# caki35/UNet-Torch

Measured on AMD Instinct MI355X. Metric: images/sec training step, 4-level U-Net 1ch→2cls 512×512, at 1/2/4/8 MI355X, higher is better.
Workload: dtype f16

## Files before the change

unet-torch_amd/csrc/kernels.h:

```cpp
#pragma once
#include "common.h"

struct ConvFwdProblem {
    int N, H, W, Ci, Co, R, S, stride, pad, Ho, Wo, ldx, ldy, in_dtype, out_dtype, flags;
    bool has_tx, has_bias, has_stats;
};
enum ConvFwdPath { FWD_MFMA3X3_F32, FWD_GEMM_F32, FWD_CONVT_F32, FWD_MFMA3X3, FWD_MFMA1X1, FWD_STEM, FWD_HEAD, FWD_SMALLK, FWD_ROOT, FWD_HEAD3, FWD_GENERIC };

bool umi_conv3x3_f32_mfma_ok(const ConvFwdProblem& p);
bool umi_gemm_f32_mfma_ok(const ConvFwdProblem& p);
bool umi_convt_f32_mfma_ok(const ConvFwdProblem& p);
bool umi_conv3x3_mfma_ok(const ConvFwdProblem& p);
bool umi_conv1x1_mfma_ok(const ConvFwdProblem& p);
bool umi_stem_fwd_ok(const ConvFwdProblem& p);
bool umi_head_fwd_ok(const ConvFwdProblem& p);
bool umi_smallk_fwd_ok(const ConvFwdProblem& p);
bool umi_root_fwd_ok(const ConvFwdProblem& p);
bool umi_head3_fwd_ok(const ConvFwdProblem& p);

constexpr int UMI_CONV_F32_OPT_IN = UMI_CONV_F32_MFMA | UMI_CONV_F32_MFMA_1X1 | UMI_CONV_F32_MFMA_2X2;
inline ConvFwdPath umi_conv_fwd_path(const ConvFwdProblem& p) {
    if (p.flags & UMI_CONV_F32_OPT_IN) {
        if (umi_conv3x3_f32_mfma_ok(p)) return FWD_MFMA3X3_F32;
        if (umi_gemm_f32_mfma_ok(p)) return FWD_GEMM_F32;
// ... 50 lines not shown
int umi_smallk_fwd_bnred(const void* x, int ldx, const void* wp, void* y, int ldy, const void* ybn, int ldybn, const void* txbn,
                         const float* rstd, float* part, long P, int Ci, int Co, hipStream_t s, float* dW = nullptr, long s_co = 0,
                         long s_ci = 0, float out_scale = 1.f, void* ws = nullptr, size_t ws_bytes = 0);
int umi_root_fwd(const ConvFwdProblem& p, const void* x, const void* wp, void* y, hipStream_t s);
int umi_head3_fwd(const ConvFwdProblem& p, const void* x, const void* tx, const void* wp, const float* bias, void* y,
                  hipStream_t s);

struct WgradProblem {
    int N, H, W, Ci, Co, R, S, stride, pad, Ho, Wo, ldx, lddy, dtype, flags;
    bool has_txa, has_txb;
};
struct WgradOut {
    float* dW; long s_co, s_ci, s_t; float out_scale;
    void* ws; size_t ws_bytes;
    umi_wgrad_pending* defer;
    float* convT_bias;
};
struct WgradBnApply { const void* y; int ldy; const void* tx_bn; const float *rstd, *sum_dz, *sum_dzx; void* dz; int lddz;
                      long count; };
enum WgradPath { WGRAD_MFMA3X3_F32, WGRAD_GEMM_F32, WGRAD_CONVT_F32, WGRAD_MFMA3X3, WGRAD_MFMA1X1, WGRAD_T, WGRAD_GATHER, WGRAD_STEM, WGRAD_HEAD, WGRAD_ROOT, WGRAD_HEAD3, WGRAD_GENERIC };

bool umi_wgrad3x3_f32_mfma_ok(const WgradProblem& p);
bool umi_wgrad_gemm_f32_mfma_ok(const WgradProblem& p);
bool umi_wgrad_convt_f32_mfma_ok(const WgradProblem& p);
bool umi_wgrad3x3_mfma_ok(const WgradProblem& p);
bool umi_wgrad1x1_mfma_ok(const WgradProblem& p);
bool umi_wgradT_mfma_ok(const WgradProblem& p);
bool umi_wgrad_gather_mfma_ok(const WgradProblem& p);
bool umi_stem_wgrad_ok(const WgradProblem& p);
bool umi_head_wgrad_ok(const WgradProblem& p);
bool umi_root_wgrad_ok(const WgradProblem& p);
bool umi_head3_wgrad_ok(const WgradProblem& p);

inline WgradPath umi_conv_wgrad_path(const WgradProblem& p) {
    if (p.flags & UMI_CONV_F32_OPT_IN) {
        if (umi_wgrad3x3_f32_mfma_ok(p)) return WGRAD_MFMA3X3_F32;
        if (umi_wgrad_gemm_f32_mfma_ok(p)) return WGRAD_GEMM_F32;
        if (umi_wgrad_convt_f32_mfma_ok(p)) return WGRAD_CONVT_F32;
        WgradProblem q = p;
        q.flags &= ~UMI_CONV_F32_OPT_IN;
        return umi_conv_wgrad_path(q);
    }
    if (umi_wgrad3x3_mfma_ok(p)) return WGRAD_MFMA3X3;
    if (umi_wgrad1x1_mfma_ok(p)) return WGRAD_MFMA1X1;
    if (umi_wgradT_mfma_ok(p)) return WGRAD_T;
    if (umi_wgrad_gather_mfma_ok(p)) return WGRAD_GATHER;
    if (umi_stem_wgrad_ok(p)) return WGRAD_STEM;
    if (umi_head_wgrad_ok(p)) return WGRAD_HEAD;
    if (umi_root_wgrad_ok(p)) return WGRAD_ROOT;
    if (umi_head3_wgrad_ok(p)) return WGRAD_HEAD3;
    return WGRAD_GENERIC;
}

size_t umi_wgrad3x3_f32_mfma_ws_bound(const WgradProblem& p);
size_t umi_wgrad_gemm_f32_mfma_ws_bound(const WgradProblem& p);
size_t umi_wgrad_convt_f32_mfma_ws_bound(const WgradProblem& p);
size_t umi_wgrad3x3_mfma_ws_bound(const WgradProblem& p);
size_t umi_wgrad1x1_mfma_ws_bound(const WgradProblem& p);
size_t umi_wgradT_mfma_ws_bound(const WgradProblem& p);
size_t umi_wgrad_gather_mfma_ws_bound(const WgradProblem& p);
size_t umi_stem_wgrad_ws_bound(const WgradProblem& p);
size_t umi_head_wgrad_ws_bound(const WgradProblem& p);
size_t umi_root_wgrad_ws_bound(const WgradProblem& p);
size_t umi_head3_wgrad_ws_bound(const WgradProblem& p);
size_t umi_conv_wgrad_generic_ws_bound(const WgradProblem& p);

// ... 77 lines not shown
```

unet-torch_amd/csrc/wgrad_mfma.hip:

```cpp
#include "kernels.h"
#include <type_traits>
#include <stdlib.h>

typedef _Float16 half8 __attribute__((ext_vector_type(8)));
typedef _Float16 half4 __attribute__((ext_vector_type(4)));
typedef short short4v __attribute__((ext_vector_type(4)));
typedef float floatx16 __attribute__((ext_vector_type(16)));

#ifdef UMI_STAMP
__device__ unsigned long long umi_stamp_buf_w[2048 * 8];
#define UMI_TW(var)                                                                       \
    unsigned long long var;                                                               \
    __builtin_amdgcn_sched_barrier(0);                                                    \
    asm volatile("s_memtime %0\n\ts_waitcnt lgkmcnt(0)" : "=s"(var)::"memory");           \
    __builtin_amdgcn_sched_barrier(0)
extern "C" int umi_debug_read_stamps_w(void* dst) {
    return (int)hipMemcpyFromSymbol(dst, HIP_SYMBOL(umi_stamp_buf_w), sizeof(umi_stamp_buf_w));
}
#endif

namespace {

constexpr int TR = 4;
constexpr int HPIX = (TR + 2) * 34;
// ... 177 lines not shown
#endif
        __syncthreads();
#ifdef UMI_STAMP
        UMI_TW(t4);
        seg[0] += t0b - t0; seg[1] += t1 - t0b; seg[2] += t2 - t1; seg[3] += t3 - t2; seg[4] += t4 - t3;
#endif
    }
#undef UMI_ISSUE
#ifdef UMI_STAMP
    UMI_TW(t_ep0);
#endif

    const int co = co0 + wco * 32 + (lane & 31);
#pragma unroll
    for (int tap = 0; tap < 9; ++tap)
#pragma unroll
        for (int r = 0; r < 16; ++r) {
            int ci = ci0 + wci * 32 + (r & 3) + 8 * (r >> 2) + 4 * (lane >> 5);
            if (ci < Ci && co < Co) part[(((long)blockIdx.y * 9 + tap) * Ci + ci) * Co + co] = acc[tap][r];
        }
#ifdef UMI_STAMP
    UMI_TW(t_end_);
    const int bid = blockIdx.y * gridDim.x + blockIdx.x;
    if (lane == 0 && bid < 512) {
#pragma unroll
        for (int i = 0; i < 5; ++i) umi_stamp_buf_w[(bid * 4 + wave) * 8 + i] = seg[i];
        umi_stamp_buf_w[(bid * 4 + wave) * 8 + 5] = t_end - t_begin;
        umi_stamp_buf_w[(bid * 4 + wave) * 8 + 6] = t_loop - t_start;
        umi_stamp_buf_w[(bid * 4 + wave) * 8 + 7] = t_end_ - t_ep0;
    }
#endif
}

constexpr int WS_SMEM = 2 * SMEM;

struct BnApply {
    const half_t* y; int ldy; const float4* tx; const float* rstd; const float* sum_dz; const float* sum_dzx; long count;
    half_t* dz; int lddz;
};

template <bool HAS_TX, bool BNA>
__global__ __launch_bounds__(512, 1) void wgrad3x3_ws_kernel(
    const half_t* __restrict__ x, int ldx, const float4* __restrict__ tx, const half_t* __restrict__ dy, int lddy,
    float* __restrict__ part, int N, int H, int W, int Ci, int Co, int tiles_x, int tiles_y, int tiles_total,
    int tiles_per_split, int n_co_t, int fast_ci, BnApply ba) {
    extern __shared__ __attribute__((aligned(16))) unsigned char smem_ws[];
    float4* txs = reinterpret_cast<float4*>(smem_ws + WS_SMEM);
    const int tid = threadIdx.x;
    const int lane = tid & 63, wave = tid >> 6;
    const bool producer = wave >= 4;
    const int n_ci_t = (int)gridDim.x / n_co_t;
    const int ci0 = (fast_ci ? (int)blockIdx.x % n_ci_t : (int)blockIdx.x / n_co_t) * 64;
    const int co0 = (fast_ci ? (int)blockIdx.x / n_ci_t : (int)blockIdx.x % n_co_t) * 64;
    const int t_begin = blockIdx.y * tiles_per_split;
    int t_end = t_begin + tiles_per_split;
    if (t_end > tiles_total) t_end = tiles_total;
    const int ntile = t_end - t_begin;
    if (HAS_TX) {
        if (tid < 64) txs[(tid & 7) * 8 + (tid >> 3)] = ci0 + tid < Ci ? tx[ci0 + tid] : make_float4(0.f, 1.f, 0.f, 0.f);
        __syncthreads();
    }

    if (producer) {
        const int ptid = tid - 256;
        const int sub = ptid & 7;
        const bool a_on = ci0 + sub * 8 < Ci, b_on = co0 + sub * 8 < Co;
        constexpr unsigned OOB = 0x7FFFFFFFu;
        int hyx[KPA], aoff[KPA];
#pragma unroll
        for (int k = 0; k < KPA; ++k) {
            int hp = (ptid >> 3) + 32 * k;
            int hy = hp / 34, hx = hp - hy * 34;
            hyx[k] = (hp < HPIX && a_on) ? (int)(((unsigned)(hy - 1) << 16) | ((unsigned)(hx - 1) & 0xffffu)) : (int)0x80000000;
            aoff[k] = (((hy - 1) * W + (hx - 1)) * ldx + ci0 + sub * 8) * 2;
        }
        const bool whole_tiles = (W & 31) == 0 && H % TR == 0;
        const int aback = (W + 1) * ldx * 2;
        int ering[KPA];
        unsigned aoffb[KPA];
#pragma unroll
        for (int k = 0; k < KPA; ++k) {
            int hp = (ptid >> 3) + 32 * k;
            int hy = hp / 34, hx = hp - hy * 34;
            ering[k] = (hp < HPIX && a_on) ? ((hx == 0 ? 1 : 0) | (hx == 33 ? 2 : 0) | (hy == 0 ? 4 : 0) | (hy == TR + 1 ? 8 : 0)) : 16;
            aoffb[k] = (unsigned)(aoff[k] + aback);
        }
        const int bcol = ptid >> 3;
        const int boff0 = (bcol * lddy + co0 + sub * 8) * 2;
        const int a_lds = (sub >> 2) * A_CHUNK + (ptid >> 3) * PROW + (sub & 3) * 16;
        const int b_lds = A_BYTES + (sub >> 2) * B_CHUNK + (ptid >> 3) * PROW + (sub & 3) * 16;
        const long ximg = (long)H * W * ldx, yimg = (long)H * W * lddy;
        float4 t[8];
#pragma unroll
        for (int j = 0; j < 8; ++j) t[j] = HAS_TX ? txs[j * 8 + sub] : make_float4(0.f, 1.f, 0.f, 0.f);
        float4 tb[8];
        float rsb[8], c1[8], c2[8];
        const long ybimg = BNA ? (long)H * W * ba.ldy : 0;
        const int ybo0 = BNA ? (bcol * ba.ldy + co0 + sub * 8) * 2 : 0;
        const bool dz_writer = BNA && ci0 == 0;
        if (BNA) {
            const float invM = 1.f / (float)ba.count;
#pragma unroll
            for (int j = 0; j < 8; ++j) {
                const int c = co0 + sub * 8 + j;
                const bool in = c < Co;
                tb[j] = in ? ba.tx[c] : make_float4(0.f, 1.f, 0.f, 0.f);
                rsb[j] = in ? ba.rstd[c] : 0.f;
                c1[j] = in ? ba.sum_dz[c] * invM : 0.f;
                c2[j] = in ? ba.sum_dzx[c] * invM : 0.f;
            }
        }
        half8 yraw0[KPB], yraw1[KPB];
        bool bvalid0[KPB], bvalid1[KPB];
        int st_n0 = 0, st_y0 = 0, st_x0 = 0, st_n1 = 0, st_y1 = 0, st_x1 = 0;
        half8 araw0[KPA], braw0[KPB], araw1[KPA], braw1[KPB];
        bool avalid0[KPA], avalid1[KPA];
        int nx_n, nx_y, nx_x;
        {
            const int tpi = tiles_x * tiles_y;
            nx_n = t_begin / tpi;
            const int rm = t_begin - nx_n * tpi;
            nx_y = (rm / tiles_x) * TR;
            nx_x = (rm % tiles_x) * 32;
        }
#ifdef UMI_EXP_WS_NO_LOAD
#define UMI_EXP_LOAD_OK(c_) ((c_) && H < 0)
#else
#define UMI_EXP_LOAD_OK(c_) (c_)
#endif
#define UMI_ISSUE_WS(S)                                                                                          \
    do {                                                                                                        \
        const __amdgpu_buffer_rsrc_t xrs = __builtin_amdgcn_make_buffer_rsrc((void*)(x + nx_n * ximg), 0, (int)(ximg * 2), 0x00020000); \
        const __amdgpu_buffer_rsrc_t yrs = __builtin_amdgcn_make_buffer_rsrc((void*)(dy + nx_n * yimg), 0, (int)(yimg * 2), 0x00020000); \
        const int org = nx_y * W + nx_x;                                                                        \
        const unsigned abase = (unsigned)org * (unsigned)(ldx * 2), bbase = (unsigned)org * (unsigned)(lddy * 2);  \
        if (whole_tiles) {                                                                                      \
            const __amdgpu_buffer_rsrc_t xrsb = __builtin_amdgcn_make_buffer_rsrc((void*)((const char*)(x + nx_n * ximg) - aback), 0, (int)(ximg * 2) + aback, 0x00020000); \
            const int edge = (nx_x == 0 ? 1 : 0) | (nx_x + 32 >= W ? 2 : 0) | (nx_y == 0 ? 4 : 0) | (nx_y + TR >= H ? 8 : 0) | 16; \
            _Pragma("unroll") for (int k = 0; k < KPA; ++k) {                                                   \
                avalid##S[k] = (ering[k] & edge) == 0;                                                          \
                araw##S[k] = __builtin_bit_cast(half8, __builtin_amdgcn_raw_buffer_load_b128(                   \
                    xrsb, UMI_EXP_LOAD_OK(avalid##S[k]) ? aoffb[k] : OOB, abase, 0));                           \
            }                                                                                                   \
        } else {                                                                                                \
            _Pragma("unroll") for (int k = 0; k < KPA; ++k) {                                                   \
                const int gy = nx_y + (hyx[k] >> 16), gx = nx_x + (int)(short)(hyx[k] & 0xffff);                \
                avalid##S[k] = hyx[k] != (int)0x80000000 && (unsigned)gy < (unsigned)H && (unsigned)gx < (unsigned)W; \
                araw##S[k] = __builtin_bit_cast(half8, __builtin_amdgcn_raw_buffer_load_b128(                   \
                    xrs, UMI_EXP_LOAD_OK(avalid##S[k]) ? abase + (unsigned)aoff[k] : OOB, 0, 0));               \
            }                                                                                                   \
        }                                                                                                       \
        _Pragma("unroll") for (int k = 0; k < KPB; ++k) {                                                       \
            const bool ok = b_on && (whole_tiles || (nx_y + k < H && nx_x + bcol < W));                         \
            braw##S[k] = __builtin_bit_cast(half8, __builtin_amdgcn_raw_buffer_load_b128(                       \
                yrs, UMI_EXP_LOAD_OK(ok) ? (unsigned)boff0 : OOB, bbase + k * W * lddy * 2, 0));                \
            if (BNA) {                                                                                          \
                const __amdgpu_buffer_rsrc_t ybrs = __builtin_amdgcn_make_buffer_rsrc((void*)(ba.y + nx_n * ybimg), 0, (int)(ybimg * 2), 0x00020000); \
                bvalid##S[k] = ok;                                                                              \
                yraw##S[k] = __builtin_bit_cast(half8, __builtin_amdgcn_raw_buffer_load_b128(                   \
                    ybrs, ok ? (unsigned)org * (unsigned)(ba.ldy * 2) + (unsigned)(ybo0 + k * W * ba.ldy * 2) : OOB, 0, 0)); \
            }                                                                                                   \
        }                                                                                                       \
        if (BNA) { st_n##S = nx_n; st_y##S = nx_y; st_x##S = nx_x; }                                            \
        nx_x += 32;                                                                                             \
        if (nx_x >= W) { nx_x = 0; nx_y += TR; if (nx_y >= H) { nx_y = 0; ++nx_n; } }                           \
    } while (0)
#ifdef UMI_EXP_WS_NO_STORE
#define UMI_STORE_WS(S, buf_)                                                                                    \
    do {                                                                                                        \
        _Pragma("unroll") for (int k = 0; k < KPA; ++k) asm volatile("" ::"v"(araw##S[k]));                     \
        _Pragma("unroll") for (int k = 0; k < KPB; ++k) asm volatile("" ::"v"(braw##S[k]));                     \
    } while (0)
#else
#define UMI_STORE_WS(S, buf_)                                                                                    \
    do {                                                                                                        \
        unsigned char* sb = smem_ws + (buf_) * SMEM;                                                            \
        if (HAS_TX) {                                                                                           \
            _Pragma("unroll") for (int k = 0; k < KPA; ++k) {                                                   \
                const half8 t8 = umi_tx8(araw##S[k], t);                                                        \
                araw##S[k] = avalid##S[k] ? t8 : araw##S[k];       \
            }                                                                                                   \
        }                                                                                                       \
        _Pragma("unroll") for (int k = 0; k < KPA; ++k)                                                         \
            if ((ptid >> 3) + 32 * k < HPIX) *reinterpret_cast<half8*>(sb + a_lds + k * 32 * PROW) = araw##S[k]; \
        if (BNA) {                                                                                              \
            _Pragma("unroll") for (int k = 0; k < KPB; ++k) {                                                   \
                const half8 o = umi_bn_dz8(yraw##S[k], braw##S[k], tb, rsb, c1, c2);    \
                braw##S[k] = bvalid##S[k] ? o : braw##S[k];              \
                if (dz_writer && bvalid##S[k])                                                                  \
                    *reinterpret_cast<half8*>(ba.dz + ((long)((long)st_n##S * H + st_y##S + k) * W + st_x##S + bcol) * ba.lddz + \
                                              co0 + sub * 8) = braw##S[k];                                      \
            }                                                                                                   \
        }                                                                                                       \
        _Pragma("unroll") for (int k = 0; k < KPB; ++k) *reinterpret_cast<half8*>(sb + b_lds + k * 32 * PROW) = braw##S[k]; \
    } while (0)
#endif

        if (ntile > 0) UMI_ISSUE_WS(0);
        if (ntile > 1) UMI_ISSUE_WS(1);
        if (ntile > 0) UMI_STORE_WS(0, 0);
        if (ntile > 2) UMI_ISSUE_WS(0);
        __syncthreads();
#ifdef UMI_STAMP
        unsigned long long pw = 0, pb = 0;
#define UMI_PS(a_) UMI_TW(a_)
#else
#define UMI_PS(a_)
#endif
        for (int i = 0; i < ntile; i += 2) {
            UMI_PS(q0);
#ifndef UMI_EXP_WS_NO_PROD
            if (i + 1 < ntile) {
                UMI_STORE_WS(1, 1);
                if (i + 3 < ntile) UMI_ISSUE_WS(1);
            }
#endif
            UMI_PS(q1);
            __syncthreads();
            UMI_PS(q2);
            if (i + 1 < ntile) {
#ifndef UMI_EXP_WS_NO_PROD
                if (i + 2 < ntile) {
                    UMI_STORE_WS(0, 0);
                    if (i + 4 < ntile) UMI_ISSUE_WS(0);
                }
#endif
                UMI_PS(q3);
                __syncthreads();
                UMI_PS(q4);
#ifdef UMI_STAMP
                pw += q3 - q2; pb += q4 - q3;
#endif
            }
#ifdef UMI_STAMP
            pw += q1 - q0; pb += q2 - q1;
#endif
        }
#ifdef UMI_STAMP
        {
            const int bid = blockIdx.y * gridDim.x + blockIdx.x;
            if (lane == 0 && bid < 256) {
                umi_stamp_buf_w[(bid * 8 + wave) * 8 + 0] = pw;
                umi_stamp_buf_w[(bid * 8 + wave) * 8 + 1] = pb;
                umi_stamp_buf_w[(bid * 8 + wave) * 8 + 5] = ntile;
            }
        }
#endif
#undef UMI_PS
#undef UMI_ISSUE_WS
#undef UMI_STORE_WS
        return;
    }

    __builtin_amdgcn_s_setprio(3);
    const int wci = wave >> 1, wco = wave & 1;
    typedef float floatx4 __attribute__((ext_vector_type(4)));
    floatx4 acc[9][2][2];
#pragma unroll
    for (int t = 0; t < 9; ++t)
#pragma unroll
        for (int ca = 0; ca < 2; ++ca)
#pragma unroll
            for (int cb = 0; cb < 2; ++cb)
#pragma unroll
                for (int r = 0; r < 4; ++r) acc[t][ca][cb][r] = 0.f;
    const int g = lane >> 4, li = lane & 15, lq = li >> 2, lp = li & 3;
    const int frag_lane = (8 * g + lq) * PROW + (4 * lp) * 2;
    __syncthreads();
#define UMI_LD_A16(dst, ca_, dx_)                                                                                \
    _Pragma("unroll") for (int rr = 0; rr < TR + 2; ++rr) dst[rr] = tr_frag(a_frag + (rr * 34 + (dx_)) * PROW + (ca_) * 32)
#define UMI_MMA16(af_, ca_, dx_)                                                                                 \
    _Pragma("unroll") for (int r = 0; r < TR; ++r)                                                              \
        _Pragma("unroll") for (int dyi = 0; dyi < 3; ++dyi)                                                     \
            _Pragma("unroll") for (int cb = 0; cb < 2; ++cb)                                                    \
                acc[dyi * 3 + (dx_)][ca_][cb] = __builtin_amdgcn_mfma_f32_16x16x32_f16(af_[r + dyi], bfr[r][cb], acc[dyi * 3 + (dx_)][ca_][cb], 0, 0, 0)
#define UMI_PIN() __builtin_amdgcn_sched_barrier(0)
#ifdef UMI_STAMP
    unsigned long long cw = 0, cb_ = 0, cstart = 0;
#endif
    for (int i = 0; i < ntile; ++i) {
#ifdef UMI_STAMP
        UMI_TW(c0);
#endif
        const unsigned char* a_frag = smem_ws + (i & 1) * SMEM + wci * A_CHUNK + frag_lane;
        const unsigned char* b_frag = smem_ws + (i & 1) * SMEM + A_BYTES + wco * B_CHUNK + frag_lane;
        half8 a0[TR + 2], a1[TR + 2], bfr[TR][2];
#pragma unroll
        for (int r = 0; r < TR; ++r)
#pragma unroll
            for (int cb = 0; cb < 2; ++cb) bfr[r][cb] = tr_frag(b_frag + (r * 32) * PROW + cb * 32);
#ifndef UMI_WS_COARSE
#define UMI_STEP(ld_, mma_) do { ld_; mma_;                                                              \
            _Pragma("unroll") for (int i_ = 0; i_ < 12; ++i_) {                                                     \
                __builtin_amdgcn_sched_group_barrier(0x008, 2, 0); __builtin_amdgcn_sched_group_barrier(0x100, 1, 0); }  \
            UMI_PIN(); } while (0)
        UMI_LD_A16(a0, 0, 0); UMI_PIN();
        UMI_STEP(UMI_LD_A16(a1, 1, 0), UMI_MMA16(a0, 0, 0));
        UMI_STEP(UMI_LD_A16(a0, 0, 1), UMI_MMA16(a1, 1, 0));
        UMI_STEP(UMI_LD_A16(a1, 1, 1), UMI_MMA16(a0, 0, 1));
        UMI_STEP(UMI_LD_A16(a0, 0, 2), UMI_MMA16(a1, 1, 1));
        UMI_STEP(UMI_LD_A16(a1, 1, 2), UMI_MMA16(a0, 0, 2));
        UMI_MMA16(a1, 1, 2);
#undef UMI_STEP
#else
        UMI_LD_A16(a0, 0, 0); UMI_PIN();
#ifdef UMI_STAMP_STEPS
        asm volatile("s_waitcnt lgkmcnt(0)" ::: "memory");
        UMI_TW(cs0);
        cstart += cs0 - c0;
#endif
        UMI_LD_A16(a1, 1, 0); UMI_PIN(); UMI_MMA16(a0, 0, 0); UMI_PIN();
        UMI_LD_A16(a0, 0, 1); UMI_PIN(); UMI_MMA16(a1, 1, 0); UMI_PIN();
        UMI_LD_A16(a1, 1, 1); UMI_PIN(); UMI_MMA16(a0, 0, 1); UMI_PIN();
        UMI_LD_A16(a0, 0, 2); UMI_PIN(); UMI_MMA16(a1, 1, 1); UMI_PIN();
        UMI_LD_A16(a1, 1, 2); UMI_PIN(); UMI_MMA16(a0, 0, 2); UMI_PIN();
        UMI_MMA16(a1, 1, 2);
#endif
#ifdef UMI_STAMP
        UMI_TW(c1);
#endif
        __syncthreads();
#ifdef UMI_STAMP
        UMI_TW(c2);
        cw += c1 - c0; cb_ += c2 - c1;
#endif
    }
#ifdef UMI_STAMP
    {
        const int bid = blockIdx.y * gridDim.x + blockIdx.x;
        if (lane == 0 && bid < 256) {
            umi_stamp_buf_w[(bid * 8 + wave) * 8 + 0] = cw;
            umi_stamp_buf_w[(bid * 8 + wave) * 8 + 1] = cb_;
            umi_stamp_buf_w[(bid * 8 + wave) * 8 + 2] = cstart;
            umi_stamp_buf_w[(bid * 8 + wave) * 8 + 5] = ntile;
        }
    }
#endif
#undef UMI_LD_A16
#undef UMI_MMA16
#undef UMI_PIN
#pragma unroll
    for (int tap = 0; tap < 9; ++tap)
#pragma unroll
        for (int ca = 0; ca < 2; ++ca)
#pragma unroll
            for (int cb = 0; cb < 2; ++cb) {
                const int co = co0 + wco * 32 + cb * 16 + (lane & 15);
#pragma unroll
                for (int r = 0; r < 4; ++r) {
                    const int ci = ci0 + wci * 32 + ca * 16 + 4 * (lane >> 4) + r;
// ... 147 lines not shown
        }
    }
#pragma unroll
    for (int hh = 0; hh < YH; ++hh) {
        const int cy = cy0 + hh * 64 + wcy * 32 + (lane & 31);
#pragma unroll
        for (int tap = 0; tap < 4; ++tap)
#pragma unroll
            for (int r = 0; r < 16; ++r) {
                int cx = cx0 + wcx * 32 + (r & 3) + 8 * (r >> 2) + 4 * (lane >> 5);
                part[(((long)blockIdx.y * 4 + tap) * Cx + cx) * Cy + cy] = acc[tap][hh][r];
            }
    }
}

void planT(int N, int h, int w, int Cx, int Cy, int* tiles_x, int* tiles_y, int* tiles_total, int* splits, int* tps) {
    *tiles_x = (w + 31) / 32;
    *tiles_y = (h + T2R - 1) / T2R;
    *tiles_total = N * (*tiles_x) * (*tiles_y);
    const long pairs = (long)(Cx / 64) * (Cy % 128 == 0 ? Cy / 128 : Cy / 64);
    static const long target2 = [] { const char* e = getenv("UMI_WGRAD_SPLIT_TARGET2"); long v = e ? atol(e) : 0; return v > 0 ? v : 1024L; }();
    long want = (target2 + pairs - 1) / pairs;
    const long slab = 4L * Cx * Cy * 4;
    long cap = (64L << 20) / slab;
    if (cap < 1) cap = 1;
    if (pairs * cap < 512 && pairs < 512) cap = (512 + pairs - 1) / pairs;
    if (want > cap) want = cap;
    if (want > *tiles_total) want = *tiles_total;
    if (want < 1) want = 1;
    *tps = (int)((*tiles_total + want - 1) / want);
    *splits = (*tiles_total + *tps - 1) / *tps;
}

void plan(int N, int H, int W, int Ci, int Co, int* tiles_x, int* tiles_y, int* tiles_total, int* splits, int* tps) {
    *tiles_x = (W + 31) / 32;
    *tiles_y = (H + TR - 1) / TR;
    *tiles_total = N * (*tiles_x) * (*tiles_y);
    const long pairs = (long)((Ci + 63) / 64) * ((Co + 63) / 64);
    static const long target = [] { const char* e = getenv("UMI_WGRAD_SPLIT_TARGET"); long v = e ? atol(e) : 0; return v > 0 ? v : 256L; }();
    long want = (target + pairs - 1) / pairs;
    const long slab = 9L * Ci * Co * 4;
    long cap = (96L << 20) / slab;
    if (cap < 1) cap = 1;
    if (pairs * cap < 256 && pairs < 256) cap = (256 + pairs - 1) / pairs;
    if (want > cap) want = cap;
    if (want > *tiles_total) want = *tiles_total;
    if (want < 1) want = 1;
    *tps = (int)((*tiles_total + want - 1) / want);
    *splits = (*tiles_total + *tps - 1) / *tps;
}

struct WGeo { int Ho, Wo, H, W, S, stride, pad; };
struct WGroup { const half_t* x[16]; const half_t* dy[16]; float* dW[16]; long s_co, s_ci; float scale; };
struct WNoGroup {};
template <int TM, bool HAS_TX, bool GATHER, bool GROUP = false>
__global__ __launch_bounds__(256, 2) void wgrad1x1_mfma_kernel(const half_t* __restrict__ x, int ldx,
                                                               const float4* __restrict__ tx,
                                                               const half_t* __restrict__ dy, int lddy,
                                                               float* __restrict__ part, long M, int Ci, int Co,
                                                               int tiles_total, int tiles_per_split, int n_co_t, WGeo geo,
                                                               typename std::conditional<GROUP, WGroup, WNoGroup>::type grp) {
    if constexpr (GROUP) { x = grp.x[blockIdx.z]; dy = grp.dy[blockIdx.z]; }
    constexpr int MT = TM / 64;
    constexpr int NCH = TM / 32;
    constexpr int CHB = 64 * PROW + 64;
    constexpr int PPP = TM / 8;
    constexpr int PXS = 256 / PPP;
    constexpr int KP = 64 / PXS;
    __shared__ __attribute__((aligned(16))) unsigned char smem[2 * NCH * CHB];
// ... 260 lines not shown
    float* const cpart = bias_out ? (float*)o.ws + (size_t)splits * 4 * Ci * Co : nullptr;
    const bool wide = Co % 128 == 0;
    const int n_cy_t = wide ? Co / 128 : Co / 64;
    dim3 grid((Ci / 64) * n_cy_t, splits), block(256);
#define UMI_GO_T(HT, YH_)                                                                                        \
    hipLaunchKernelGGL((wgradT2x2_mfma_kernel<HT, YH_>), grid, block, 0, s, (const half_t*)x, p.ldx, (const half_t*)dy, p.lddy, \
                       (const float4*)txb, (float*)o.ws, N, Ho, Wo, Ci, Co, tiles_x, tiles_y, tiles_total, tps, n_cy_t, cpart)
    if (txb) { if (wide) UMI_GO_T(true, 2); else UMI_GO_T(true, 1); }
    else { if (wide) UMI_GO_T(false, 2); else UMI_GO_T(false, 1); }
#undef UMI_GO_T
    if (bias_out) {
        UMI_LAUNCH_CHECK();
        umi_launch_reduce_rows2(cpart, splits, Ci, bias_out, nullptr, o.out_scale, s);
    }
    UMI_LAUNCH_CHECK();
    umi_launch_wgrad_reduce(splits, 4, Ci, Co, o, s);
    UMI_LAUNCH_CHECK();
    return UMI_OK;
}

bool umi_wgrad3x3_mfma_ok(const WgradProblem& p) {
    if (p.flags & UMI_CONV_FORCE_GENERIC) return false;
    if (p.dtype != UMI_F16 || p.has_txb) return false;
    if (p.R != 3 || p.S != 3 || p.stride != 1 || p.pad != 1 || p.Ho != p.H || p.Wo != p.W) return false;
    if (p.Ci % 8 || p.Co % 8 || p.ldx % 8 || p.lddy % 8) return false;
    if ((long)p.H * p.W * (p.ldx > p.lddy ? p.ldx : p.lddy) * 2 >= 0x7FFFFFF0L) return false;
    return true;
}
size_t umi_wgrad3x3_mfma_ws_bound(const WgradProblem& facts) {
    WgradProblem p = facts;
    p.H = p.Ho; p.W = p.Wo; p.stride = p.pad = 1; p.ldx = p.lddy = 8;
    if (!umi_wgrad3x3_mfma_ok(p)) return 0;
    int tx_, ty_, tt, splits, tps;
    plan(p.N, p.H, p.W, p.Ci, p.Co, &tx_, &ty_, &tt, &splits, &tps);
    return (size_t)splits * 9 * p.Ci * p.Co * sizeof(float);
}

int umi_wgrad3x3_mfma(const WgradProblem& p, const void* x, const void* txa, const void* dy, const WgradOut& o, hipStream_t s,
                      const WgradBnApply* bna) {
    const int N = p.N, H = p.H, W = p.W, Ci = p.Ci, Co = p.Co, ldx = p.ldx, lddy = p.lddy;
    void* const ws = o.ws;
    int tiles_x, tiles_y, tiles_total, splits, tps;
    plan(N, H, W, Ci, Co, &tiles_x, &tiles_y, &tiles_total, &splits, &tps);
    if (o.ws_bytes < (size_t)splits * 9 * Ci * Co * sizeof(float)) return UMI_ERR_WORKSPACE;
    if (((uintptr_t)x | (uintptr_t)dy) & 15) return UMI_ERR_BADARG;
    const int n_co_t = (Co + 63) / 64;
    dim3 grid(((Ci + 63) / 64) * n_co_t, splits), block(256);
    static const int force_fast = [] { const char* e = getenv("UMI_WGRAD_FAST_CI"); return e ? atoi(e) : -1; }();
    const int fast_ci = force_fast >= 0 ? force_fast : (Co < 1.59 * Ci ? 1 : 0);
    static const bool classic = [] { const char* e = getenv("UMI_WGRAD_CLASSIC"); return e && e[0] == '1'; }();
    if (bna && classic) return UMI_ERR_UNSUPPORTED;
    if (!classic) {
        constexpr int dyn = WS_SMEM + 64 * (int)sizeof(float4);
        static const int attr_rc = [] {
            int a = (int)hipFuncSetAttribute((const void*)wgrad3x3_ws_kernel<true, false>, hipFuncAttributeMaxDynamicSharedMemorySize, dyn);
            int b = (int)hipFuncSetAttribute((const void*)wgrad3x3_ws_kernel<false, false>, hipFuncAttributeMaxDynamicSharedMemorySize, dyn);
            int c = (int)hipFuncSetAttribute((const void*)wgrad3x3_ws_kernel<true, true>, hipFuncAttributeMaxDynamicSharedMemorySize, dyn);
            int d = (int)hipFuncSetAttribute((const void*)wgrad3x3_ws_kernel<false, true>, hipFuncAttributeMaxDynamicSharedMemorySize, dyn);
            return a ? a : (b ? b : (c ? c : d));
        }();
        if (attr_rc) return attr_rc;
        dim3 block_ws(512);
        const BnApply ba = bna ? BnApply{(const half_t*)bna->y, bna->ldy, (const float4*)bna->tx_bn, bna->rstd, bna->sum_dz, bna->sum_dzx,
                                         bna->count, (half_t*)bna->dz, bna->lddz}
                               : BnApply{nullptr, 0, nullptr, nullptr, nullptr, nullptr, 1, nullptr, 0};
#define GO_WS(HT, BN_)                                                                                              \
        hipLaunchKernelGGL((wgrad3x3_ws_kernel<HT, BN_>), grid, block_ws, dyn, s, (const half_t*)x, ldx, (const float4*)txa,   \
                           (const half_t*)dy, lddy, (float*)ws, N, H, W, Ci, Co, tiles_x, tiles_y, tiles_total, tps, n_co_t, fast_ci, ba)
        if (bna) { if (txa) GO_WS(true, true); else GO_WS(false, true); }
        else { if (txa) GO_WS(true, false); else GO_WS(false, false); }
#undef GO_WS
    } else if (txa)
        hipLaunchKernelGGL(wgrad3x3_mfma_kernel<true>, grid, block, 0, s, (const half_t*)x, ldx, (const float4*)txa,
                           (const half_t*)dy, lddy, (float*)ws, N, H, W, Ci, Co, tiles_x, tiles_y, tiles_total, tps,
                           n_co_t, fast_ci);
    else
        hipLaunchKernelGGL(wgrad3x3_mfma_kernel<false>, grid, block, 0, s, (const half_t*)x, ldx, (const float4*)txa,
                           (const half_t*)dy, lddy, (float*)ws, N, H, W, Ci, Co, tiles_x, tiles_y, tiles_total, tps,
                           n_co_t, fast_ci);
    UMI_LAUNCH_CHECK();
    umi_launch_wgrad_reduce(splits, 9, Ci, Co, o, s);
    UMI_LAUNCH_CHECK();
    return UMI_OK;
}
```

Baseline: 761.1.

## Add tall 8-row tiles to warp-specialized 3x3 wgrad kernel

Templates the warp-specialized 3x3 weight-gradient kernel on the number of 4-row half tiles (NH), letting one pipeline stage hold an 8-row tile. The halo rows between the two halves are loaded once and shared, which cuts redundant input loads and halves the number of barrier stages per pixel row. By default the tall path runs only for W==32 layers with an even tiles-per-split, keeping the same split order. It can also be forced with an environment variable. The cost is larger shared-memory buffers and a more complex producer/consumer schedule.

```diff
diff --git a/unet-torch_amd/csrc/kernels.h b/unet-torch_amd/csrc/kernels.h
--- a/unet-torch_amd/csrc/kernels.h
+++ b/unet-torch_amd/csrc/kernels.h
@@ -106,6 +106,9 @@
 bool umi_root_wgrad_ok(const WgradProblem& p);
 bool umi_head3_wgrad_ok(const WgradProblem& p);
 
+inline bool umi_wgrad3x3_tall_tiles(const WgradProblem& p) { return p.W % 32 == 0 && p.H % 8 == 0; }
+inline bool umi_wgrad3x3_tall_same_order(const WgradProblem& p) { return p.W == 32 && p.H % 8 == 0; }
+
 inline WgradPath umi_conv_wgrad_path(const WgradProblem& p) {
     if (p.flags & UMI_CONV_F32_OPT_IN) {
         if (umi_wgrad3x3_f32_mfma_ok(p)) return WGRAD_MFMA3X3_F32;
diff --git a/unet-torch_amd/csrc/wgrad_mfma.hip b/unet-torch_amd/csrc/wgrad_mfma.hip
--- a/unet-torch_amd/csrc/wgrad_mfma.hip
+++ b/unet-torch_amd/csrc/wgrad_mfma.hip
@@ -233,20 +233,34 @@
 #endif
 }
 
-constexpr int WS_SMEM = 2 * SMEM;
+template <int NH>
+struct WsTile {
+    static constexpr int ROWS = NH * TR;
+    static constexpr int UROWS = NH == 1 ? TR + 2 : TR + 1;
+    static constexpr int UPIX = UROWS * 34;
+    static constexpr int KPA = (UPIX * 8 + 255) / 256;
+    static constexpr int A_CHUNK = (ROWS + 2) * 34 * PROW + 64;
+    static constexpr int A_BYTES = 2 * A_CHUNK;
+    static constexpr int B_CHUNK = ROWS * 32 * PROW + 64;
+    static constexpr int BUF = A_BYTES + 2 * B_CHUNK;
+    static constexpr int SMEM = 2 * BUF;
+};
 
 struct BnApply {
     const half_t* y; int ldy; const float4* tx; const float* rstd; const float* sum_dz; const float* sum_dzx; long count;
     half_t* dz; int lddz;
 };
 
-template <bool HAS_TX, bool BNA>
+template <bool HAS_TX, bool BNA, int NH>
 __global__ __launch_bounds__(512, 1) void wgrad3x3_ws_kernel(
     const half_t* __restrict__ x, int ldx, const float4* __restrict__ tx, const half_t* __restrict__ dy, int lddy,
     float* __restrict__ part, int N, int H, int W, int Ci, int Co, int tiles_x, int tiles_y, int tiles_total,
     int tiles_per_split, int n_co_t, int fast_ci, BnApply ba) {
+    typedef WsTile<NH> T;
+    constexpr int ROWS = T::ROWS, UROWS = T::UROWS, UPIX = T::UPIX, KPA = T::KPA, A_CHUNK = T::A_CHUNK, A_BYTES = T::A_BYTES,
+                  B_CHUNK = T::B_CHUNK, SMEM = T::BUF;
     extern __shared__ __attribute__((aligned(16))) unsigned char smem_ws[];
-    float4* txs = reinterpret_cast<float4*>(smem_ws + WS_SMEM);
+    float4* txs = reinterpret_cast<float4*>(smem_ws + T::SMEM);
     const int tid = threadIdx.x;
     const int lane = tid & 63, wave = tid >> 6;
     const bool producer = wave >= 4;
@@ -272,10 +286,10 @@
         for (int k = 0; k < KPA; ++k) {
             int hp = (ptid >> 3) + 32 * k;
             int hy = hp / 34, hx = hp - hy * 34;
-            hyx[k] = (hp < HPIX && a_on) ? (int)(((unsigned)(hy - 1) << 16) | ((unsigned)(hx - 1) & 0xffffu)) : (int)0x80000000;
+            hyx[k] = (hp < UPIX && a_on) ? (int)(((unsigned)(hy - 1) << 16) | ((unsigned)(hx - 1) & 0xffffu)) : (int)0x80000000;
             aoff[k] = (((hy - 1) * W + (hx - 1)) * ldx + ci0 + sub * 8) * 2;
         }
-        const bool whole_tiles = (W & 31) == 0 && H % TR == 0;
+        const bool whole_tiles = NH == 2 || ((W & 31) == 0 && H % TR == 0);
         const int aback = (W + 1) * ldx * 2;
         int ering[KPA];
         unsigned aoffb[KPA];
@@ -283,7 +297,7 @@
         for (int k = 0; k < KPA; ++k) {
             int hp = (ptid >> 3) + 32 * k;
             int hy = hp / 34, hx = hp - hy * 34;
-            ering[k] = (hp < HPIX && a_on) ? ((hx == 0 ? 1 : 0) | (hx == 33 ? 2 : 0) | (hy == 0 ? 4 : 0) | (hy == TR + 1 ? 8 : 0)) : 16;
+            ering[k] = (hp < UPIX && a_on) ? ((hx == 0 ? 1 : 0) | (hx == 33 ? 2 : 0) | (hy == 0 ? 4 : 0) | (hy == UROWS - 1 ? 8 : 0)) : 16;
             aoffb[k] = (unsigned)(aoff[k] + aback);
         }
         const int bcol = ptid >> 3;
@@ -321,7 +335,7 @@
             const int tpi = tiles_x * tiles_y;
             nx_n = t_begin / tpi;
             const int rm = t_begin - nx_n * tpi;
-            nx_y = (rm / tiles_x) * TR;
+            nx_y = (rm / tiles_x) * ROWS;
             nx_x = (rm % tiles_x) * 32;
         }
 #ifdef UMI_EXP_WS_NO_LOAD
@@ -329,7 +343,7 @@
 #else
 #define UMI_EXP_LOAD_OK(c_) (c_)
 #endif
-#define UMI_ISSUE_WS(S)                                                                                          \
+#define UMI_ISSUE_WS(S, HF)                                                                                       \
     do {                                                                                                        \
         const __amdgpu_buffer_rsrc_t xrs = __builtin_amdgcn_make_buffer_rsrc((void*)(x + nx_n * ximg), 0, (int)(ximg * 2), 0x00020000); \
         const __amdgpu_buffer_rsrc_t yrs = __builtin_amdgcn_make_buffer_rsrc((void*)(dy + nx_n * yimg), 0, (int)(yimg * 2), 0x00020000); \
@@ -337,11 +351,12 @@
         const unsigned abase = (unsigned)org * (unsigned)(ldx * 2), bbase = (unsigned)org * (unsigned)(lddy * 2);  \
         if (whole_tiles) {                                                                                      \
             const __amdgpu_buffer_rsrc_t xrsb = __builtin_amdgcn_make_buffer_rsrc((void*)((const char*)(x + nx_n * ximg) - aback), 0, (int)(ximg * 2) + aback, 0x00020000); \
-            const int edge = (nx_x == 0 ? 1 : 0) | (nx_x + 32 >= W ? 2 : 0) | (nx_y == 0 ? 4 : 0) | (nx_y + TR >= H ? 8 : 0) | 16; \
+            const int edge = (nx_x == 0 ? 1 : 0) | (nx_x + 32 >= W ? 2 : 0) | ((HF) == 0 && nx_y == 0 ? 4 : 0) |                \
+                             ((HF) == NH - 1 && nx_y + ROWS >= H ? 8 : 0) | 16;                                         \
             _Pragma("unroll") for (int k = 0; k < KPA; ++k) {                                                   \
                 avalid##S[k] = (ering[k] & edge) == 0;                                                          \
                 araw##S[k] = __builtin_bit_cast(half8, __builtin_amdgcn_raw_buffer_load_b128(                   \
-                    xrsb, UMI_EXP_LOAD_OK(avalid##S[k]) ? aoffb[k] : OOB, abase, 0));                           \
+                    xrsb, UMI_EXP_LOAD_OK(avalid##S[k]) ? aoffb[k] : OOB, abase + (HF) * UROWS * W * ldx * 2, 0)); \
             }                                                                                                   \
         } else {                                                                                                \
             _Pragma("unroll") for (int k = 0; k < KPA; ++k) {                                                   \
@@ -354,28 +369,30 @@
         _Pragma("unroll") for (int k = 0; k < KPB; ++k) {                                                       \
             const bool ok = b_on && (whole_tiles || (nx_y + k < H && nx_x + bcol < W));                         \
             braw##S[k] = __builtin_bit_cast(half8, __builtin_amdgcn_raw_buffer_load_b128(                       \
-                yrs, UMI_EXP_LOAD_OK(ok) ? (unsigned)boff0 : OOB, bbase + k * W * lddy * 2, 0));                \
+                yrs, UMI_EXP_LOAD_OK(ok) ? (unsigned)boff0 : OOB, bbase + ((HF) * TR + k) * W * lddy * 2, 0)); \
             if (BNA) {                                                                                          \
                 const __amdgpu_buffer_rsrc_t ybrs = __builtin_amdgcn_make_buffer_rsrc((void*)(ba.y + nx_n * ybimg), 0, (int)(ybimg * 2), 0x00020000); \
                 bvalid##S[k] = ok;                                                                              \
                 yraw##S[k] = __builtin_bit_cast(half8, __builtin_amdgcn_raw_buffer_load_b128(                   \
-                    ybrs, ok ? (unsigned)org * (unsigned)(ba.ldy * 2) + (unsigned)(ybo0 + k * W * ba.ldy * 2) : OOB, 0, 0)); \
+                    ybrs, ok ? (unsigned)org * (unsigned)(ba.ldy * 2) + (unsigned)(ybo0 + ((HF) * TR + k) * W * ba.ldy * 2) : OOB, 0, 0)); \
             }                                                                                                   \
         }                                                                                                       \
-        if (BNA) { st_n##S = nx_n; st_y##S = nx_y; st_x##S = nx_x; }                                            \
-        nx_x += 32;                                                                                             \
-        if (nx_x >= W) { nx_x = 0; nx_y += TR; if (nx_y >= H) { nx_y = 0; ++nx_n; } }                           \
+        if (BNA) { st_n##S = nx_n; st_y##S = nx_y + (HF) * TR; st_x##S = nx_x; }                                \
+        if ((HF) == NH - 1) {                                                                                   \
+            nx_x += 32;                                                                                         \
+            if (nx_x >= W) { nx_x = 0; nx_y += ROWS; if (nx_y >= H) { nx_y = 0; ++nx_n; } }                     \
+        }                                                                                                       \
     } while (0)
 #ifdef UMI_EXP_WS_NO_STORE
-#define UMI_STORE_WS(S, buf_)                                                                                    \
+#define UMI_STORE_WS(S, buf_, HF)                                                                                 \
     do {                                                                                                        \
         _Pragma("unroll") for (int k = 0; k < KPA; ++k) asm volatile("" ::"v"(araw##S[k]));                     \
         _Pragma("unroll") for (int k = 0; k < KPB; ++k) asm volatile("" ::"v"(braw##S[k]));                     \
     } while (0)
 #else
-#define UMI_STORE_WS(S, buf_)                                                                                    \
+#define UMI_STORE_WS(S, buf_, HF)                                                                                 \
     do {                                                                                                        \
-        unsigned char* sb = smem_ws + (buf_) * SMEM;                                                            \
+        unsigned char* sb = smem_ws + (buf_) * SMEM;           \
         if (HAS_TX) {                                                                                           \
             _Pragma("unroll") for (int k = 0; k < KPA; ++k) {                                                   \
                 const half8 t8 = umi_tx8(araw##S[k], t);                                                        \
@@ -383,7 +400,7 @@
             }                                                                                                   \
         }                                                                                                       \
         _Pragma("unroll") for (int k = 0; k < KPA; ++k)                                                         \
-            if ((ptid >> 3) + 32 * k < HPIX) *reinterpret_cast<half8*>(sb + a_lds + k * 32 * PROW) = araw##S[k]; \
+            if ((ptid >> 3) + 32 * k < UPIX) *reinterpret_cast<half8*>(sb + a_lds + ((HF) * UPIX + k * 32) * PROW) = araw##S[k]; \
         if (BNA) {                                                                                              \
             _Pragma("unroll") for (int k = 0; k < KPB; ++k) {                                                   \
                 const half8 o = umi_bn_dz8(yraw##S[k], braw##S[k], tb, rsb, c1, c2);    \
@@ -393,49 +410,79 @@
                                               co0 + sub * 8) = braw##S[k];                                      \
             }                                                                                                   \
         }                                                                                                       \
-        _Pragma("unroll") for (int k = 0; k < KPB; ++k) *reinterpret_cast<half8*>(sb + b_lds + k * 32 * PROW) = braw##S[k]; \
+        _Pragma("unroll") for (int k = 0; k < KPB; ++k) *reinterpret_cast<half8*>(sb + b_lds + ((HF) * TR + k) * 32 * PROW) = braw##S[k]; \
     } while (0)
 #endif
 
-        if (ntile > 0) UMI_ISSUE_WS(0);
-        if (ntile > 1) UMI_ISSUE_WS(1);
-        if (ntile > 0) UMI_STORE_WS(0, 0);
-        if (ntile > 2) UMI_ISSUE_WS(0);
-        __syncthreads();
 #ifdef UMI_STAMP
         unsigned long long pw = 0, pb = 0;
 #define UMI_PS(a_) UMI_TW(a_)
 #else
 #define UMI_PS(a_)
 #endif
-        for (int i = 0; i < ntile; i += 2) {
-            UMI_PS(q0);
+        if constexpr (NH == 1) {
+            if (ntile > 0) UMI_ISSUE_WS(0, 0);
+            if (ntile > 1) UMI_ISSUE_WS(1, 0);
+            if (ntile > 0) UMI_STORE_WS(0, 0, 0);
+            if (ntile > 2) UMI_ISSUE_WS(0, 0);
+            __syncthreads();
+            for (int i = 0; i < ntile; i += 2) {
+                UMI_PS(q0);
 #ifndef UMI_EXP_WS_NO_PROD
-            if (i + 1 < ntile) {
-                UMI_STORE_WS(1, 1);
-                if (i + 3 < ntile) UMI_ISSUE_WS(1);
-            }
-#endif
-            UMI_PS(q1);
+                if (i + 1 < ntile) {
+                    UMI_STORE_WS(1, 1, 0);
+                    if (i + 3 < ntile) UMI_ISSUE_WS(1, 0);
+                }
+#endif
+                UMI_PS(q1);
+                __syncthreads();
+                UMI_PS(q2);
+                if (i + 1 < ntile) {
+#ifndef UMI_EXP_WS_NO_PROD
+                    if (i + 2 < ntile) {
+                        UMI_STORE_WS(0, 0, 0);
+                        if (i + 4 < ntile) UMI_ISSUE_WS(0, 0);
+                    }
+#endif
+                    UMI_PS(q3);
+                    __syncthreads();
+                    UMI_PS(q4);
+#ifdef UMI_STAMP
+                    pw += q3 - q2; pb += q4 - q3;
+#endif
+                }
+#ifdef UMI_STAMP
+                pw += q1 - q0; pb += q2 - q1;
+#endif
+            }
+        } else {
+            if (ntile > 0) {
+                UMI_ISSUE_WS(0, 0);
+                UMI_ISSUE_WS(1, 1);
+                UMI_STORE_WS(0, 0, 0);
+                if (ntile > 1) UMI_ISSUE_WS(0, 0);
+                UMI_STORE_WS(1, 0, 1);
+                if (ntile > 1) UMI_ISSUE_WS(1, 1);
+            }
             __syncthreads();
-            UMI_PS(q2);
-            if (i + 1 < ntile) {
+            for (int i = 0; i < ntile; ++i) {
+                UMI_PS(q0);
 #ifndef UMI_EXP_WS_NO_PROD
-                if (i + 2 < ntile) {
-                    UMI_STORE_WS(0, 0);
-                    if (i + 4 < ntile) UMI_ISSUE_WS(0);
+                if (i + 1 < ntile) {
+                    const int nb = (i + 1) & 1;
+                    UMI_STORE_WS(0, nb, 0);
+                    if (i + 2 < ntile) UMI_ISSUE_WS(0, 0);
+                    UMI_STORE_WS(1, nb, 1);
+                    if (i + 2 < ntile) UMI_ISSUE_WS(1, 1);
                 }
 #endif
-                UMI_PS(q3);
+                UMI_PS(q1);
                 __syncthreads();
-                UMI_PS(q4);
-#ifdef UMI_STAMP
-                pw += q3 - q2; pb += q4 - q3;
-#endif
-            }
-#ifdef UMI_STAMP
-            pw += q1 - q0; pb += q2 - q1;
-#endif
+                UMI_PS(q2);
+#ifdef UMI_STAMP
+                pw += q1 - q0; pb += q2 - q1;
+#endif
+            }
         }
 #ifdef UMI_STAMP
         {
@@ -483,40 +530,72 @@
 #ifdef UMI_STAMP
         UMI_TW(c0);
 #endif
-        const unsigned char* a_frag = smem_ws + (i & 1) * SMEM + wci * A_CHUNK + frag_lane;
-        const unsigned char* b_frag = smem_ws + (i & 1) * SMEM + A_BYTES + wco * B_CHUNK + frag_lane;
+        const unsigned char* a_tile = smem_ws + (i & 1) * SMEM + wci * A_CHUNK + frag_lane;
+        const unsigned char* b_tile = smem_ws + (i & 1) * SMEM + A_BYTES + wco * B_CHUNK + frag_lane;
         half8 a0[TR + 2], a1[TR + 2], bfr[TR][2];
-#pragma unroll
-        for (int r = 0; r < TR; ++r)
-#pragma unroll
-            for (int cb = 0; cb < 2; ++cb) bfr[r][cb] = tr_frag(b_frag + (r * 32) * PROW + cb * 32);
+#define UMI_LD_B16(r_, base_)                                                                                    \
+    _Pragma("unroll") for (int cb = 0; cb < 2; ++cb) bfr[r_][cb] = tr_frag((base_) + ((r_) * 32) * PROW + cb * 32)
+#pragma unroll
+        for (int hf = 0; hf < NH; ++hf) {
+            const unsigned char* a_frag = a_tile + hf * TR * 34 * PROW;
+            const unsigned char* b_frag = b_tile + hf * TR * 32 * PROW;
 #ifndef UMI_WS_COARSE
 #define UMI_STEP(ld_, mma_) do { ld_; mma_;                                                              \
             _Pragma("unroll") for (int i_ = 0; i_ < 12; ++i_) {                                                     \
                 __builtin_amdgcn_sched_group_barrier(0x008, 2, 0); __builtin_amdgcn_sched_group_barrier(0x100, 1, 0); }  \
             UMI_PIN(); } while (0)
-        UMI_LD_A16(a0, 0, 0); UMI_PIN();
-        UMI_STEP(UMI_LD_A16(a1, 1, 0), UMI_MMA16(a0, 0, 0));
-        UMI_STEP(UMI_LD_A16(a0, 0, 1), UMI_MMA16(a1, 1, 0));
-        UMI_STEP(UMI_LD_A16(a1, 1, 1), UMI_MMA16(a0, 0, 1));
-        UMI_STEP(UMI_LD_A16(a0, 0, 2), UMI_MMA16(a1, 1, 1));
-        UMI_STEP(UMI_LD_A16(a1, 1, 2), UMI_MMA16(a0, 0, 2));
-        UMI_MMA16(a1, 1, 2);
+            if (hf == 0) {
+#pragma unroll
+                for (int r = 0; r < TR; ++r) UMI_LD_B16(r, b_frag);
+                UMI_LD_A16(a0, 0, 0); UMI_PIN();
+            }
+            UMI_STEP(UMI_LD_A16(a1, 1, 0), UMI_MMA16(a0, 0, 0));
+            UMI_STEP(UMI_LD_A16(a0, 0, 1), UMI_MMA16(a1, 1, 0));
+            UMI_STEP(UMI_LD_A16(a1, 1, 1), UMI_MMA16(a0, 0, 1));
+            UMI_STEP(UMI_LD_A16(a0, 0, 2), UMI_MMA16(a1, 1, 1));
+            UMI_STEP(UMI_LD_A16(a1, 1, 2), UMI_MMA16(a0, 0, 2));
+            if (hf + 1 < NH) {
+                const unsigned char* a_nx = a_frag + TR * 34 * PROW;
+                const unsigned char* b_nx = b_frag + TR * 32 * PROW;
+#pragma unroll
+                for (int r = 0; r < TR; ++r) {
+#pragma unroll
+                    for (int dyi = 0; dyi < 3; ++dyi)
+#pragma unroll
+                        for (int cb = 0; cb < 2; ++cb)
+                            acc[dyi * 3 + 2][1][cb] = __builtin_amdgcn_mfma_f32_16x16x32_f16(a1[r + dyi], bfr[r][cb], acc[dyi * 3 + 2][1][cb], 0, 0, 0);
+#pragma unroll
+                    for (int rr = (r < 2 ? 2 * r : r + 2); rr < (r < 2 ? 2 * r + 2 : r + 3); ++rr) a0[rr] = tr_frag(a_nx + (rr * 34) * PROW);
+                    if (r > 0) UMI_LD_B16(r - 1, b_nx);
+#pragma unroll
+                    for (int i_ = 0; i_ < 6; ++i_) {
+                        __builtin_amdgcn_sched_group_barrier(0x008, 1, 0); __builtin_amdgcn_sched_group_barrier(0x100, 1, 0); }
+                    __builtin_amdgcn_sched_group_barrier(0x100, 2, 0);
+                    UMI_PIN();
+                }
+                UMI_LD_B16(TR - 1, b_nx); UMI_PIN();
+            } else {
+                UMI_MMA16(a1, 1, 2);
+            }
 #undef UMI_STEP
 #else
-        UMI_LD_A16(a0, 0, 0); UMI_PIN();
+#pragma unroll
+            for (int r = 0; r < TR; ++r) UMI_LD_B16(r, b_frag);
+            UMI_LD_A16(a0, 0, 0); UMI_PIN();
 #ifdef UMI_STAMP_STEPS
-        asm volatile("s_waitcnt lgkmcnt(0)" ::: "memory");
-        UMI_TW(cs0);
-        cstart += cs0 - c0;
-#endif
-        UMI_LD_A16(a1, 1, 0); UMI_PIN(); UMI_MMA16(a0, 0, 0); UMI_PIN();
-        UMI_LD_A16(a0, 0, 1); UMI_PIN(); UMI_MMA16(a1, 1, 0); UMI_PIN();
-        UMI_LD_A16(a1, 1, 1); UMI_PIN(); UMI_MMA16(a0, 0, 1); UMI_PIN();
-        UMI_LD_A16(a0, 0, 2); UMI_PIN(); UMI_MMA16(a1, 1, 1); UMI_PIN();
-        UMI_LD_A16(a1, 1, 2); UMI_PIN(); UMI_MMA16(a0, 0, 2); UMI_PIN();
-        UMI_MMA16(a1, 1, 2);
-#endif
+            asm volatile("s_waitcnt lgkmcnt(0)" ::: "memory");
+            UMI_TW(cs0);
+            if (hf == 0) cstart += cs0 - c0;
+#endif
+            UMI_LD_A16(a1, 1, 0); UMI_PIN(); UMI_MMA16(a0, 0, 0); UMI_PIN();
+            UMI_LD_A16(a0, 0, 1); UMI_PIN(); UMI_MMA16(a1, 1, 0); UMI_PIN();
+            UMI_LD_A16(a1, 1, 1); UMI_PIN(); UMI_MMA16(a0, 0, 1); UMI_PIN();
+            UMI_LD_A16(a0, 0, 2); UMI_PIN(); UMI_MMA16(a1, 1, 1); UMI_PIN();
+            UMI_LD_A16(a1, 1, 2); UMI_PIN(); UMI_MMA16(a0, 0, 2); UMI_PIN();
+            UMI_MMA16(a1, 1, 2);
+#endif
+        }
+#undef UMI_LD_B16
 #ifdef UMI_STAMP
         UMI_TW(c1);
 #endif
@@ -730,9 +809,9 @@
     *splits = (*tiles_total + *tps - 1) / *tps;
 }
 
-void plan(int N, int H, int W, int Ci, int Co, int* tiles_x, int* tiles_y, int* tiles_total, int* splits, int* tps) {
+void plan(int N, int H, int W, int Ci, int Co, int rows, int* tiles_x, int* tiles_y, int* tiles_total, int* splits, int* tps) {
     *tiles_x = (W + 31) / 32;
-    *tiles_y = (H + TR - 1) / TR;
+    *tiles_y = (H + rows - 1) / rows;
     *tiles_total = N * (*tiles_x) * (*tiles_y);
     const long pairs = (long)((Ci + 63) / 64) * ((Co + 63) / 64);
     static const long target = [] { const char* e = getenv("UMI_WGRAD_SPLIT_TARGET"); long v = e ? atol(e) : 0; return v > 0 ? v : 256L; }();
@@ -1059,7 +1138,12 @@
     p.H = p.Ho; p.W = p.Wo; p.stride = p.pad = 1; p.ldx = p.lddy = 8;
     if (!umi_wgrad3x3_mfma_ok(p)) return 0;
     int tx_, ty_, tt, splits, tps;
-    plan(p.N, p.H, p.W, p.Ci, p.Co, &tx_, &ty_, &tt, &splits, &tps);
+    plan(p.N, p.H, p.W, p.Ci, p.Co, TR, &tx_, &ty_, &tt, &splits, &tps);
+    if (umi_wgrad3x3_tall_tiles(p)) {
+        int splits8;
+        plan(p.N, p.H, p.W, p.Ci, p.Co, 2 * TR, &tx_, &ty_, &tt, &splits8, &tps);
+        if (splits8 > splits) splits = splits8;
+    }
     return (size_t)splits * 9 * p.Ci * p.Co * sizeof(float);
 }
 
@@ -1067,36 +1151,49 @@
                       const WgradBnApply* bna) {
     const int N = p.N, H = p.H, W = p.W, Ci = p.Ci, Co = p.Co, ldx = p.ldx, lddy = p.lddy;
     void* const ws = o.ws;
+    static const bool classic = [] { const char* e = getenv("UMI_WGRAD_CLASSIC"); return e && e[0] == '1'; }();
+    static const bool tile4 = [] { const char* e = getenv("UMI_WGRAD_TILE4"); return e && e[0] == '1'; }();
+    static const bool tile8 = [] { const char* e = getenv("UMI_WGRAD_TILE8"); return e && e[0] == '1'; }();
+    bool tall = !classic && !tile4 && tile8 && umi_wgrad3x3_tall_tiles(p);
     int tiles_x, tiles_y, tiles_total, splits, tps;
-    plan(N, H, W, Ci, Co, &tiles_x, &tiles_y, &tiles_total, &splits, &tps);
+    plan(N, H, W, Ci, Co, tall ? 2 * TR : TR, &tiles_x, &tiles_y, &tiles_total, &splits, &tps);
+    if (!classic && !tile4 && !tall && umi_wgrad3x3_tall_same_order(p) && tps % 2 == 0) {
+        tall = true;
+        tiles_y /= 2; tiles_total /= 2; tps /= 2;
+    }
     if (o.ws_bytes < (size_t)splits * 9 * Ci * Co * sizeof(float)) return UMI_ERR_WORKSPACE;
     if (((uintptr_t)x | (uintptr_t)dy) & 15) return UMI_ERR_BADARG;
     const int n_co_t = (Co + 63) / 64;
     dim3 grid(((Ci + 63) / 64) * n_co_t, splits), block(256);
     static const int force_fast = [] { const char* e = getenv("UMI_WGRAD_FAST_CI"); return e ? atoi(e) : -1; }();
     const int fast_ci = force_fast >= 0 ? force_fast : (Co < 1.59 * Ci ? 1 : 0);
-    static const bool classic = [] { const char* e = getenv("UMI_WGRAD_CLASSIC"); return e && e[0] == '1'; }();
     if (bna && classic) return UMI_ERR_UNSUPPORTED;
     if (!classic) {
-        constexpr int dyn = WS_SMEM + 64 * (int)sizeof(float4);
+        constexpr int txs_bytes = 64 * (int)sizeof(float4);
         static const int attr_rc = [] {
-            int a = (int)hipFuncSetAttribute((const void*)wgrad3x3_ws_kernel<true, false>, hipFuncAttributeMaxDynamicSharedMemorySize, dyn);
-            int b = (int)hipFuncSetAttribute((const void*)wgrad3x3_ws_kernel<false, false>, hipFuncAttributeMaxDynamicSharedMemorySize, dyn);
-            int c = (int)hipFuncSetAttribute((const void*)wgrad3x3_ws_kernel<true, true>, hipFuncAttributeMaxDynamicSharedMemorySize, dyn);
-            int d = (int)hipFuncSetAttribute((const void*)wgrad3x3_ws_kernel<false, true>, hipFuncAttributeMaxDynamicSharedMemorySize, dyn);
-            return a ? a : (b ? b : (c ? c : d));
+            int rc = 0;
+#define UMI_DYN_WS(HT, BN_, NH_)                                                                                    \
+            if (!rc) rc = (int)hipFuncSetAttribute((const void*)wgrad3x3_ws_kernel<HT, BN_, NH_>, hipFuncAttributeMaxDynamicSharedMemorySize, \
+                                                   WsTile<NH_>::SMEM + txs_bytes)
+            UMI_DYN_WS(true, false, 1); UMI_DYN_WS(false, false, 1); UMI_DYN_WS(true, true, 1); UMI_DYN_WS(false, true, 1);
+            UMI_DYN_WS(true, false, 2); UMI_DYN_WS(false, false, 2); UMI_DYN_WS(true, true, 2); UMI_DYN_WS(false, true, 2);
+#undef UMI_DYN_WS
+            return rc;
         }();
         if (attr_rc) return attr_rc;
         dim3 block_ws(512);
         const BnApply ba = bna ? BnApply{(const half_t*)bna->y, bna->ldy, (const float4*)bna->tx_bn, bna->rstd, bna->sum_dz, bna->sum_dzx,
                                          bna->count, (half_t*)bna->dz, bna->lddz}
                                : BnApply{nullptr, 0, nullptr, nullptr, nullptr, nullptr, 1, nullptr, 0};
-#define GO_WS(HT, BN_)                                                                                              \
-        hipLaunchKernelGGL((wgrad3x3_ws_kernel<HT, BN_>), grid, block_ws, dyn, s, (const half_t*)x, ldx, (const float4*)txa,   \
-                           (const half_t*)dy, lddy, (float*)ws, N, H, W, Ci, Co, tiles_x, tiles_y, tiles_total, tps, n_co_t, fast_ci, ba)
+#define GO_WS_(HT, BN_, NH_)                                                                                        \
+        hipLaunchKernelGGL((wgrad3x3_ws_kernel<HT, BN_, NH_>), grid, block_ws, WsTile<NH_>::SMEM + txs_bytes, s, (const half_t*)x, ldx, \
+                           (const float4*)txa, (const half_t*)dy, lddy, (float*)ws, N, H, W, Ci, Co, tiles_x, tiles_y, tiles_total, tps, \
+                           n_co_t, fast_ci, ba)
+#define GO_WS(HT, BN_) do { if (tall) GO_WS_(HT, BN_, 2); else GO_WS_(HT, BN_, 1); } while (0)
         if (bna) { if (txa) GO_WS(true, true); else GO_WS(false, true); }
         else { if (txa) GO_WS(true, false); else GO_WS(false, false); }
 #undef GO_WS
+#undef GO_WS_
     } else if (txa)
         hipLaunchKernelGGL(wgrad3x3_mfma_kernel<true>, grid, block, 0, s, (const half_t*)x, ldx, (const float4*)txa,
                            (const half_t*)dy, lddy, (float*)ws, N, H, W, Ci, Co, tiles_x, tiles_y, tiles_total, tps,
```

New measurement: 760.7. About the same (-0.1%).
